# hanquansanren/DvD

Hardware: AMD Instinct MI355X
Metric: documents/sec (50-step DDIM, 288x288 grid) (higher is better)
Workload: dtype f16

## Files before the change

dvd_amd/csrc/tokens.hip:

```cpp
#include "common.h"
#include "mfma.h"

namespace dvd {

__device__ __forceinline__ float wave_sum(float v) {
#pragma unroll
  for (int o = 32; o > 0; o >>= 1) v += __shfl_xor(v, o);
  return v;
}

__global__ void __launch_bounds__(256) embed_obs_ln_kernel(const float* __restrict__ x, const float* __restrict__ w,
                                                           const float* __restrict__ bias,
                                                           const float* __restrict__ pos, float* __restrict__ tok32,
                                                           _Float16* __restrict__ ln16, int g, long rows) {
  const long row = (long)blockIdx.x * 4 + (threadIdx.x >> 6);
  if (row >= rows) return;
  const int lane = threadIdx.x & 63;
  const int side = g >> 1, T = side * side;
  const int n = (int)(row / T), t = (int)(row % T);
  const int ty = t / side, tx = t % side;
  float pv[8];
#pragma unroll
  for (int c = 0; c < 2; ++c)
#pragma unroll
    for (int p = 0; p < 2; ++p)
#pragma unroll
      for (int q = 0; q < 2; ++q)
        pv[c * 4 + p * 2 + q] = x[(((size_t)n * 2 + c) * g + (2 * ty + p)) * g + 2 * tx + q];
  float v[6];
  float s = 0.f;
#pragma unroll
  for (int j = 0; j < 6; ++j) {
    const int o = lane + 64 * j;
    float acc = bias[o];
#pragma unroll
    for (int k = 0; k < 8; ++k) acc += w[o * 8 + k] * pv[k];
    acc += pos[(size_t)t * 384 + o];
    v[j] = acc;
    s += acc;
  }
  const float mean = wave_sum(s) * (1.f / 384.f);
  float q2 = 0.f;
#pragma unroll
  for (int j = 0; j < 6; ++j) {
    const float d = v[j] - mean;
    q2 += d * d;
  }
  const float rstd = rsqrtf(wave_sum(q2) * (1.f / 384.f) + 1e-6f);
#pragma unroll
  for (int j = 0; j < 6; ++j) {
    const int o = lane + 64 * j;
    tok32[row * 384 + o] = v[j];
    ln16[row * 384 + o] = (_Float16)((v[j] - mean) * rstd);
  }
}

template <int C>
__global__ void __launch_bounds__(256) layernorm_rows_kernel(const float* __restrict__ in, int ldin, long sIn,
                                                             _Float16* __restrict__ out, int ldout, long sOut,
                                                             const float* __restrict__ gamma,
                                                             const float* __restrict__ beta,
                                                             const float* __restrict__ shift,
                                                             const float* __restrict__ scale, int ldmod,
                                                             int mod_rows, float eps, long rows) {
  constexpr int PER = C / 64;
  constexpr int V = (C == 384) ? 2 : 4;
  constexpr int NV = PER / V;
  const long row = (long)blockIdx.x * 4 + (threadIdx.x >> 6);
  if (row >= rows) return;
  const int lane = threadIdx.x & 63;
  const float* ip = in + blockIdx.y * sIn + row * ldin;
  float v[PER];
  float s = 0.f;
  typedef float fvec __attribute__((ext_vector_type(V)));
  typedef _Float16 hvec __attribute__((ext_vector_type(V)));
#pragma unroll
  for (int k = 0; k < NV; ++k) {
    const int c0 = (k * 64 + lane) * V;
    const fvec x = *(const fvec*)(ip + c0);
#pragma unroll
    for (int e = 0; e < V; ++e) {
      v[k * V + e] = x[e];
// ... 450 lines not shown
    }
  }
}

__global__ void __launch_bounds__(256) final_tokens_kernel(const float* __restrict__ z,
                                                           const float* __restrict__ gamma,
                                                           const float* __restrict__ beta,
                                                           const float* __restrict__ shift,
                                                           const float* __restrict__ scale, int ldmod,
                                                           int mod_rows, const float* __restrict__ w,
                                                           const float* __restrict__ b,
                                                           const float* __restrict__ init_flow,
                                                           float* __restrict__ x0, float* __restrict__ tok8, int g,
                                                           long rows) {
  constexpr int C = 1536, PER = 24;
  const long row = (long)blockIdx.x * 4 + (threadIdx.x >> 6);
  if (row >= rows) return;
  const int lane = threadIdx.x & 63;
  const float* ip = z + row * C;
  float v[PER];
  float s = 0.f;
#pragma unroll
  for (int k = 0; k < 6; ++k) {
    const floatx4 f = *(const floatx4*)(ip + (k * 64 + lane) * 4);
#pragma unroll
    for (int e = 0; e < 4; ++e) {
      v[k * 4 + e] = f[e];
      s += f[e];
    }
  }
  float mean = wave_sum(s) * (1.f / C);
  float q2 = 0.f;
#pragma unroll
  for (int k = 0; k < PER; ++k) {
    const float d = v[k] - mean;
    q2 += d * d;
  }
  float rstd = rsqrtf(wave_sum(q2) * (1.f / C) + 1e-5f);
  s = 0.f;
#pragma unroll
  for (int k = 0; k < 6; ++k)
#pragma unroll
    for (int e = 0; e < 4; ++e) {
      const int c = (k * 64 + lane) * 4 + e;
      v[k * 4 + e] = (v[k * 4 + e] - mean) * rstd * gamma[c] + beta[c];
      s += v[k * 4 + e];
    }
  mean = wave_sum(s) * (1.f / C);
  q2 = 0.f;
#pragma unroll
  for (int k = 0; k < PER; ++k) {
    const float d = v[k] - mean;
    q2 += d * d;
  }
  rstd = rsqrtf(wave_sum(q2) * (1.f / C) + 1e-6f);
  const float* sh = shift + (row / mod_rows) * ldmod;
  const float* sc = scale + (row / mod_rows) * ldmod;
  float dot[8];
#pragma unroll
  for (int j = 0; j < 8; ++j) dot[j] = 0.f;
#pragma unroll
  for (int k = 0; k < 6; ++k)
#pragma unroll
    for (int e = 0; e < 4; ++e) {
      const int c = (k * 64 + lane) * 4 + e;
      const float y = ((v[k * 4 + e] - mean) * rstd) * (1.f + sc[c]) + sh[c];
#pragma unroll
      for (int j = 0; j < 8; ++j) dot[j] += y * w[j * C + c];
    }
#pragma unroll
  for (int j = 0; j < 8; ++j) dot[j] = wave_sum(dot[j]);
  if (lane < 8) {
    float o = 0.f;
#pragma unroll
    for (int j = 0; j < 8; ++j)
      if (lane == j) o = dot[j];
    o += b[lane];
    if (tok8) tok8[row * 8 + lane] = o;
    const int side = g >> 1, T = side * side;
    const int n = (int)(row / T), t = (int)(row % T);
    const int p = lane >> 2, q = (lane >> 1) & 1, c = lane & 1;
    const size_t at = (((size_t)n * 2 + c) * g + 2 * (t / side) + p) * g + 2 * (t % side) + q;
    x0[at] = o + (init_flow ? init_flow[at] : 0.f);
  }
}

}

using namespace dvd;

#define LAUNCH_ROWS(rows) cdiv((rows), 4), 256, 0, (hipStream_t)stream

extern "C" int dvd_embed_obs_ln(const float* x, const float* w, const float* bias, const float* pos, float* tok32,
                                void* ln16, int n, int g, void* stream) {
  DVD_REQUIRE(x && w && bias && pos && tok32 && ln16, "embed_obs_ln: null pointer");
  DVD_REQUIRE(n > 0 && g >= 2 && g % 2 == 0, "embed_obs_ln: bad shape");
  const long rows = (long)n * (g / 2) * (g / 2);
  embed_obs_ln_kernel<<<LAUNCH_ROWS(rows)>>>(x, w, bias, pos, tok32, (_Float16*)ln16, g, rows);
  return check_launch("embed_obs_ln");
}

extern "C" int dvd_layernorm_rows(const float* in, int ldin, long stride_in, void* out16, int ldout, long stride_out,
                                  int batch, long rows, int c, const float* gamma, const float* beta,
                                  const float* shift, const float* scale, int ldmod, int mod_rows, float eps,
                                  void* stream) {
  DVD_REQUIRE(in && out16, "layernorm_rows: null pointer");
  DVD_REQUIRE(c == 384 || c == 1536, "layernorm_rows: C=%d not in {384,1536}", c);
  DVD_REQUIRE((gamma == nullptr) == (beta == nullptr) && (shift == nullptr) == (scale == nullptr),
              "layernorm_rows: affine / modulate pointers must come in pairs");
  DVD_REQUIRE(!shift || mod_rows > 0, "layernorm_rows: mod_rows");
  DVD_REQUIRE(rows > 0 && batch > 0 && batch < 65536, "layernorm_rows: bad rows/batch");
  DVD_REQUIRE(ldin % 4 == 0 && stride_in % 2 == 0 && ldout % 4 == 0 && stride_out % 2 == 0 && ldmod % 4 == 0 &&
                  ((uintptr_t)in % 16) == 0 && ((uintptr_t)out16 % 8) == 0 && ((uintptr_t)gamma % 16) == 0 &&
                  ((uintptr_t)beta % 16) == 0 && ((uintptr_t)shift % 16) == 0 && ((uintptr_t)scale % 16) == 0,
              "layernorm_rows: rows must be 16-byte aligned (vector loads)");
  dim3 grid(cdiv(rows, 4), batch);
  if (c == 384)
    layernorm_rows_kernel<384><<<grid, 256, 0, (hipStream_t)stream>>>(in, ldin, stride_in, (_Float16*)out16, ldout,
                                                                       stride_out, gamma, beta, shift, scale, ldmod,
                                                                       mod_rows > 0 ? mod_rows : 1, eps, rows);
  else
    layernorm_rows_kernel<1536><<<grid, 256, 0, (hipStream_t)stream>>>(in, ldin, stride_in, (_Float16*)out16, ldout,
                                                                        stride_out, gamma, beta, shift, scale, ldmod,
                                                                        mod_rows > 0 ? mod_rows : 1, eps, rows);
  return check_launch("layernorm_rows");
}

extern "C" int dvd_build_r_rows(const float* feat_nhwc, const float* init_feat_nchw, const float* flow, void* out16,
                                int ldo, int n, int g, int n_hyp, int mode, void* stream) {
  DVD_REQUIRE(feat_nhwc && flow && out16, "build_r_rows: null pointer");
  DVD_REQUIRE(ldo >= 1032 && n > 0 && g >= 2 && g % 2 == 0 && n_hyp > 0 && mode >= 0 && mode <= 3,
              "build_r_rows: bad arguments");
  DVD_REQUIRE(mode != 3 || init_feat_nchw, "build_r_rows: mode 3 needs init_feat");
  const long items = (long)n * (g / 2) * (g / 2) * 4;
  build_r_rows_kernel<<<LAUNCH_ROWS(items)>>>(feat_nhwc, init_feat_nchw, flow, (_Float16*)out16, ldo, g, n_hyp, mode,
                                              items);
  return check_launch("build_r_rows");
}

extern "C" int dvd_patch_rows(const float* in, long sn, long sc, long sy, long sx, float* out, int ldo, int n, int c,
                              int g, void* stream) {
  DVD_REQUIRE(in && out, "patch_rows: null pointer");
  DVD_REQUIRE(n > 0 && c > 0 && g >= 2 && g % 2 == 0 && ldo >= 4 * c, "patch_rows: bad shape");
  const long total = (long)n * (g / 2) * (g / 2) * 4 * c;
  patch_rows_kernel<<<cdiv(total, 256), 256, 0, (hipStream_t)stream>>>(in, sn, sc, sy, sx, out, ldo, c, g, total);
  return check_launch("patch_rows");
}

extern "C" int dvd_dwconv3x3(const void* in16, void* out16, const float* w9c, const float* b, int n, int side, int c,
                             void* stream) {
  DVD_REQUIRE(in16 && out16 && w9c && b, "dwconv3x3: null pointer");
  DVD_REQUIRE(n > 0 && side > 0 && c % 8 == 0, "dwconv3x3: bad shape");
#ifdef DVD_LAB
  if (getenv("DVD_DWCONV_V1")) {
    const long total1 = (long)n * side * side * (c / 8);
    dwconv3x3_kernel<<<cdiv(total1, 256), 256, 0, (hipStream_t)stream>>>((const _Float16*)in16, (_Float16*)out16, w9c, b,
                                                                         side, c, total1);
    return check_launch("dwconv3x3(lab v1)");
  }
#endif
  int stx = (c % 512 == 0 && (long)n * side * side >= 16384) ? 3 : 0, ssy = 24;
  bool snt = true;
  (void)snt;
#ifdef DVD_LAB
  if (getenv("DVD_DWCONV_TY") || getenv("DVD_DWCONV_TX")) stx = 0;
  if (const char* e = getenv("DVD_DWCONV_STRIP")) stx = (c % 512 == 0) ? atoi(e) : 0;
  if (const char* e = getenv("DVD_DWCONV_SY")) ssy = atoi(e);
  if (const char* e = getenv("DVD_DWCONV_NT")) snt = atoi(e) != 0;
#endif
  if (stx >= 2 && stx <= 4 && ssy >= 1) {
    const int xstrips = cdiv(side, stx), ybands = cdiv(side, ssy);
    const int nwaves = n * ybands * xstrips * (c / 512);
    const dim3 g(cdiv(nwaves, 4));
#define DW_STRIP(TX_, NT_) dwconv3x3_strip_kernel<TX_, NT_><<<g, 256, 0, (hipStream_t)stream>>>((const _Float16*)in16, (_Float16*)out16, w9c, b, side, c, ssy, xstrips, ybands, nwaves)
#ifdef DVD_LAB
    if (stx == 2) { if (snt) DW_STRIP(2, true); else DW_STRIP(2, false); }
    else if (stx == 4) { if (snt) DW_STRIP(4, true); else DW_STRIP(4, false); }
    else if (!snt) DW_STRIP(3, false);
    else
#endif
    DW_STRIP(3, true);
#undef DW_STRIP
    return check_launch("dwconv3x3(strip)");
  }
  int ty = DW_TY_P, tx = DW_TX_P;
#ifdef DVD_LAB
  if (const char* e = getenv("DVD_DWCONV_TY")) ty = atoi(e);
  if (const char* e = getenv("DVD_DWCONV_TX")) tx = atoi(e);
#endif
  const long total = (long)n * cdiv(side, ty) * cdiv(side, tx) * (c / 8);
  const dim3 grd(cdiv(total, 256));
#define DW_LAUNCH(TX_, TY_) dwconv3x3_tile_kernel<TX_, TY_><<<grd, 256, 0, (hipStream_t)stream>>>((const _Float16*)in16, (_Float16*)out16, w9c, b, side, c, total)
#ifdef DVD_LAB
  if (tx == 2 && ty == 2) DW_LAUNCH(2, 2);
  else if (tx == 2 && ty == 4) DW_LAUNCH(2, 4);
  else if (tx == 2 && ty == 8) DW_LAUNCH(2, 8);
  else if (tx == 1 && ty == 4) DW_LAUNCH(1, 4);
  else if (tx == 1 && ty == 8) DW_LAUNCH(1, 8);
  else if (tx == 2) DW_LAUNCH(2, 1);
  else if (ty == 1) DW_LAUNCH(4, 1);
  else if (ty == 4) DW_LAUNCH(4, 4);
  else
#endif
  DW_LAUNCH(DW_TX_P, DW_TY_P);
#undef DW_LAUNCH
  return check_launch("dwconv3x3");
}

extern "C" int dvd_colmean(const float* z, float* partial, float* pooled, int n, int t, int c, int chunks,
                           void* stream) {
  DVD_REQUIRE(z && partial && pooled, "colmean: null pointer");
  DVD_REQUIRE(n > 0 && n < 65536 && t > 0 && c > 0 && chunks > 0 && chunks < 65536, "colmean: bad shape");
  dim3 grid(cdiv(c, 256), chunks, n);
  colsum_partial_kernel<<<grid, 256, 0, (hipStream_t)stream>>>(z, partial, t, c, chunks);
  colmean_final_kernel<<<cdiv((long)n * c, 256), 256, 0, (hipStream_t)stream>>>(partial, pooled, t, c, chunks, n * c);
  return check_launch("colmean");
}

extern "C" int dvd_posenc_add(float* z, const float* hs, const float* ws, const float* htab, const float* wtab,
                              int n, int side, int c, void* stream) {
  DVD_REQUIRE(z && hs && ws && htab && wtab, "posenc_add: null pointer");
  DVD_REQUIRE(n > 0 && side > 0 && c % 4 == 0, "posenc_add: bad shape");
  const long total4 = (long)n * side * side * (c / 4);
  posenc_add_kernel<<<cdiv(total4, 256), 256, 0, (hipStream_t)stream>>>(z, hs, ws, htab, wtab, side, c, total4);
  return check_launch("posenc_add");
}

extern "C" int dvd_small_linear(const float* x, int ldx, const float* w, const float* b, float* y, int ldy, int m,
                                int k, int n, int kmod, int act_in, int act_out, void* stream) {
  DVD_REQUIRE(x && w && y, "small_linear: null pointer");
  DVD_REQUIRE(m > 0 && k > 0 && n > 0 && kmod > 0 && act_in >= 0 && act_in <= 2 && act_out >= 0 && act_out <= 3,
              "small_linear: bad arguments");
  small_linear_kernel<<<dim3(cdiv(n, 4), cdiv(m, 8)), 256, 0, (hipStream_t)stream>>>(x, ldx, w, b, y, ldy, m, k, n, kmod, act_in,
                                                                                       act_out);
  return check_launch("small_linear");
}

extern "C" int dvd_final_tokens(const float* z, const float* gamma, const float* beta, const float* shift,
                                const float* scale, int ldmod, int mod_rows, const float* w8, const float* b8,
                                const float* init_flow, float* x0, float* tok8, int n, int g, void* stream) {
  DVD_REQUIRE(z && gamma && beta && shift && scale && w8 && b8 && x0, "final_tokens: null pointer");
  DVD_REQUIRE(n > 0 && g >= 2 && g % 2 == 0 && mod_rows > 0, "final_tokens: bad shape");
  const long rows = (long)n * (g / 2) * (g / 2);
  final_tokens_kernel<<<LAUNCH_ROWS(rows)>>>(z, gamma, beta, shift, scale, ldmod, mod_rows, w8, b8, init_flow, x0,
                                             tok8, g, rows);
  return check_launch("final_tokens");
}
```

dvd_amd/lib.py:

```python
from __future__ import annotations

import ctypes as C
import os

import torch

_HERE = os.path.dirname(os.path.abspath(__file__))
LIB_PATH = os.path.join(_HERE, "libdvd_hip.so")


class DvdError(RuntimeError):
    pass


def _load():
    if not os.path.exists(LIB_PATH):
        raise DvdError(
            f"{LIB_PATH} is missing: build it with `python -c 'import __graft_entry__ as g; g.build()'` "
            "or `make -C dvd_amd/csrc`.  The DvD engine has no non-HIP fallback.")
    return C.CDLL(LIB_PATH)


_lib = _load()

# ... 30 lines not shown
                ("O", C.c_void_p), ("ldo", C.c_int), ("strideO", C.c_long),
                ("scale", C.c_float)]


class CnOp(C.Structure):
    _fields_ = [("op", C.c_int), ("a", C.c_int), ("b", C.c_int), ("dst", C.c_int), ("ks", C.c_int), ("dil", C.c_int),
                ("cout", C.c_int), ("act", C.c_int), ("w_off", C.c_long), ("h", C.c_int), ("w", C.c_int),
                ("flag", C.c_int)]


class RaggedImage(C.Structure):
    _fields_ = [("src", C.c_void_p), ("out", C.c_void_p), ("h", C.c_int), ("w", C.c_int)]


SSIM_REPLICATE, SSIM_VALID = 0, 1
MSSSIM_DOCUNET, MSSSIM_WANG = 0, 1

PNG_SEGMENT = 32768
PNG_HUFFMAN_FIXED, PNG_HUFFMAN_DYNAMIC = 0, 1

JPEG_420, JPEG_444 = 0, 1


class JpegDecInfo(C.Structure):
    _fields_ = [("h", C.c_int), ("w", C.c_int), ("out_h", C.c_int), ("out_w", C.c_int), ("components", C.c_int),
                ("hs", C.c_int), ("vs", C.c_int), ("orientation", C.c_int), ("restart_interval", C.c_int),
                ("scan_offset", C.c_long), ("scan_bytes", C.c_long), ("blocks", C.c_long), ("scratch_bytes", C.c_long)]


JPEG_DECODE_CODES = {-20: "HEADER", -21: "PROGRESSIVE", -22: "EXTENDED", -23: "LOSSLESS", -24: "ARITHMETIC", -25: "PRECISION",
                     -26: "COMPONENTS", -27: "ADOBE", -28: "SAMPLING", -29: "SCANS", -30: "QUANT16", -31: "TABLE", -32: "SIZE",
                     -33: "ORIENTATION", -34: "NOSYNC", -35: "DATA"}
JPEGDEC_SUBSEQ = 128

class SflowParams(C.Structure):
    _fields_ = [(name, C.c_int) for name in ("levels", "w_top", "w", "iters_top", "iters", "alpha", "d", "gamma", "T", "eps")]


SFLOW_DEFAULTS = dict(levels=4, w_top=10, w=2, iters_top=60, iters=30, alpha=510, d=10200, gamma=1, T=8160, eps=1 << 17)
SFLOW_MIN_TOP = 12

RAGGED_CAP = 64

NON_STATUS = {"dvd_last_error", "dvd_version", "dvd_engine_workspace_bytes", "dvd_engine_tensor_count",
              "dvd_flash_attn_kernel_name", "dvd_gemm_kernel_name", "dvd_convnet_workspace_bytes", "dvd_convnet_weight_floats",
              "dvd_ingest_scratch_bytes", "dvd_ingest_ragged_scratch_bytes", "dvd_resize_gray_scratch_bytes",
              "dvd_msssim_workspace_bytes", "dvd_png_bound", "dvd_png_scratch_bytes", "dvd_png_scratch_bytes_huff", "dvd_jpeg_bound",
              "dvd_jpeg_scratch_bytes", "dvd_sflow_level_workspace_bytes", "dvd_sflow_workspace_bytes",
              "dvd_adist_workspace_bytes"}

SIGNATURES = {
    "dvd_grid_sample_bilinear_zeros_ac": [c_void, c_void, c_void, C.c_int, C.c_int, C.c_int, C.c_int, C.c_int,
                                          C.c_int, C.c_int, c_void],
    "dvd_unwarp_f32": [c_void, C.c_int, c_void, c_void, C.c_int, C.c_int, C.c_float, c_void],
    "dvd_unwarp_u8": [c_void, C.c_int, c_void, c_void, C.c_int, C.c_int, C.c_float, c_void],
    "dvd_unwarp_f32_batch": [c_void, C.c_int, c_void, c_void, C.c_int, C.c_int, C.c_int, C.c_float, c_void],
    "dvd_unwarp_u8_batch": [c_void, C.c_int, c_void, c_void, C.c_int, C.c_int, C.c_int, C.c_float, c_void],
    "dvd_unwarp_grid": [c_void, C.c_int, c_void, C.c_int, C.c_int, C.c_float, c_void],
    "dvd_unwarp_u8_ragged": [c_void, C.c_int, C.POINTER(RaggedImage), C.c_int, C.c_float, c_void],
    "dvd_grid_sample_bicubic_zeros_ac": [c_void, c_void, c_void, C.c_int, C.c_int, C.c_int, C.c_int, C.c_int,
                                         C.c_int, C.c_int, c_void],
    "dvd_unwarp_u8_bicubic_batch": [c_void, C.c_int, c_void, c_void, C.c_int, C.c_int, C.c_int, C.c_float, c_void],
    "dvd_unwarp_u8_bicubic_ragged": [c_void, C.c_int, C.POINTER(RaggedImage), C.c_int, C.c_float, c_void],
    "dvd_sched_step": [C.POINTER(SchedCoef), c_void, c_void, c_void, c_void, c_void, C.c_int, C.c_int, c_void],
    "dvd_sched_step_clip": [C.POINTER(SchedCoef), c_void, c_void, c_void, c_void, c_void, C.c_int, C.c_int, c_void],
    "dvd_hyp_mean_clamp": [c_void, c_void, C.c_int, C.c_int, C.c_int, c_void],
    "dvd_selftest_mfma": [c_void, c_void, c_void, c_void, c_void],
    "dvd_gemm_nt": [C.POINTER(GemmDesc), c_void],
    "dvd_gemm_kernel_name": [C.POINTER(GemmDesc)],
    "dvd_flash_attn": [C.POINTER(AttnDesc), c_void],
    "dvd_embed_obs_ln": [c_void, c_void, c_void, c_void, c_void, c_void, C.c_int, C.c_int, c_void],
    "dvd_layernorm_rows": [c_void, C.c_int, C.c_long, c_void, C.c_int, C.c_long, C.c_int, C.c_long, C.c_int, c_void,
                           c_void, c_void, c_void, C.c_int, C.c_int, C.c_float, c_void],
    "dvd_build_r_rows": [c_void, c_void, c_void, c_void, C.c_int, C.c_int, C.c_int, C.c_int, C.c_int, c_void],
    "dvd_patch_rows": [c_void, C.c_long, C.c_long, C.c_long, C.c_long, c_void, C.c_int, C.c_int, C.c_int, C.c_int,
                       c_void],
    "dvd_dwconv3x3": [c_void, c_void, c_void, c_void, C.c_int, C.c_int, C.c_int, c_void],
    "dvd_colmean": [c_void, c_void, c_void, C.c_int, C.c_int, C.c_int, C.c_int, c_void],
    "dvd_posenc_add": [c_void, c_void, c_void, c_void, c_void, C.c_int, C.c_int, C.c_int, c_void],
    "dvd_small_linear": [c_void, C.c_int, c_void, c_void, c_void, C.c_int, C.c_int, C.c_int, C.c_int, C.c_int, C.c_int,
                         C.c_int, c_void],
    "dvd_final_tokens": [c_void, c_void, c_void, c_void, c_void, C.c_int, C.c_int, c_void, c_void, c_void, c_void,
                         c_void, C.c_int, C.c_int, c_void],
    "dvd_im2col3x3": [c_void, C.c_long, C.c_long, C.c_long, c_void, C.c_int, C.c_int, C.c_int, C.c_int, c_void],
    "dvd_conv3x3_nhwc": [c_void, C.c_int, c_void, C.c_int, c_void, c_void, C.c_int, C.c_int, C.c_int, C.c_int, c_void],
    "dvd_maxpool2_nhwc": [c_void, c_void, C.c_int, C.c_int, C.c_int, c_void],
    "dvd_resize_bilinear_nhwc": [c_void, c_void, C.c_int, C.c_int, C.c_int, C.c_int, C.c_int, c_void],
    "dvd_nhwc_to_nchw": [c_void, c_void, C.c_int, C.c_int, C.c_int, c_void],
    "dvd_convnet_create": [C.POINTER(CnOp), C.c_int, C.c_int, C.c_int, C.c_int, C.c_int, C.POINTER(c_void)],
    "dvd_convnet_create_batched": [C.POINTER(CnOp), C.c_int, C.c_int, C.c_int, C.c_int, C.c_int, C.c_int, C.POINTER(c_void)],
    "dvd_convnet_destroy": [c_void],
    "dvd_convnet_slot_shape": [c_void, C.c_int, C.POINTER(C.c_int), C.POINTER(C.c_int), C.POINTER(C.c_int)],
    "dvd_convnet_run": [c_void, c_void, c_void, c_void, C.c_long, C.c_int, C.POINTER(C.c_int), C.POINTER(c_void), c_void],
    "dvd_resize_bilinear_nchw": [c_void, c_void, C.c_long, C.c_int, C.c_int, C.c_int, C.c_int, C.c_int, c_void],
    "dvd_threshold_mask_mul": [c_void, c_void, c_void, c_void, C.c_int, C.c_long, C.c_float, c_void],
    "dvd_threshold_mask_mul_batch": [c_void, c_void, c_void, c_void, C.c_int, C.c_int, C.c_long, C.c_float, c_void],
    "dvd_flash_attn_f32": [C.POINTER(AttnDesc), c_void],
    "dvd_layernorm256_f32": [c_void, c_void, C.c_long, c_void, c_void, C.c_float, c_void],
    "dvd_add_rows_f32": [c_void, c_void, c_void, C.c_long, C.c_int, C.c_int, c_void],
    "dvd_transpose_f32": [c_void, c_void, C.c_int, C.c_int, C.c_int, c_void],
    "dvd_soft_mask_mul_batch": [c_void, c_void, c_void, C.c_int, C.c_int, C.c_long, c_void],
    "dvd_convex_upsample": [c_void, c_void, C.c_int, C.c_int, C.c_int, c_void, c_void, C.c_int, C.c_float, c_void],
    "dvd_ingest_u8": [c_void, C.c_int, C.c_int, C.c_int, c_void, C.c_int, c_void, c_void, c_void],
    "dvd_ingest_ragged_scratch_bytes": [C.c_int, C.c_int],
    "dvd_ingest_u8_ragged": [C.POINTER(RaggedImage), C.c_int, C.c_int, c_void, C.c_int, c_void, c_void],
    "dvd_resize_gray_scratch_bytes": [C.c_int, C.c_int, C.c_int, C.c_int],
    "dvd_resize_gray_u8": [c_void, C.c_int, C.c_int, C.c_int, c_void, C.c_int, C.c_int, c_void, c_void],
    "dvd_ssim_scale": [c_void, c_void, C.c_int, C.c_int, C.c_int, C.c_int, c_void, c_void],
    "dvd_ssim_finalize": [c_void, C.c_int, C.c_int, C.c_long, c_void, C.c_int, c_void],
    "dvd_reduce2_pair": [c_void, c_void, c_void, c_void, C.c_int, C.c_int, C.c_int, C.c_int, c_void],
    "dvd_msssim_workspace_bytes": [C.c_int, C.c_int, C.c_int],
    "dvd_msssim_scales": [c_void, c_void, C.c_int, C.c_int, C.c_int, C.c_int, c_void, c_void, c_void],
    "dvd_dsift_u8": [c_void, C.c_int, C.c_int, C.c_int, C.c_int, c_void, c_void],
    "dvd_sflow_cost": [c_void, c_void, c_void, C.c_int, C.c_int, C.c_int, C.POINTER(SflowParams), c_void, c_void],
    "dvd_sflow_level_workspace_bytes": [C.c_int, C.c_int, C.c_int],
    "dvd_sflow_level": [c_void, c_void, c_void, C.c_int, C.c_int, C.c_int, C.c_int, C.POINTER(SflowParams), c_void, c_void, c_void,
                        c_void],
    "dvd_sflow_workspace_bytes": [C.c_int, C.c_int, C.POINTER(SflowParams)],
    "dvd_sflow": [c_void, c_void, C.c_int, C.c_int, C.c_int, C.POINTER(SflowParams), c_void, c_void, c_void, c_void],
    "dvd_ad_fit": [c_void, C.c_int, C.c_int, C.c_int, c_void, c_void, c_void, c_void],
    "dvd_ad_align": [c_void, c_void, C.c_int, C.c_int, C.c_int, c_void, c_void],
    "dvd_ad_weighted": [c_void, c_void, C.c_int, C.c_int, C.c_int, c_void, c_void, c_void],
    "dvd_adist_workspace_bytes": [C.c_int, C.c_int, C.POINTER(SflowParams)],
    "dvd_adist": [c_void, c_void, C.c_int, C.c_int, C.c_int, C.POINTER(SflowParams), c_void, c_void, c_void, c_void, c_void, c_void,
                  c_void, c_void, c_void],
    "dvd_png_bound": [C.c_int, C.c_int],
    "dvd_png_scratch_bytes": [C.c_int, C.c_int],
    "dvd_png_encode_rgb8": [c_void, C.c_int, C.c_int, c_void, C.c_long, c_void, c_void, c_void],
    "dvd_png_scratch_bytes_huff": [C.c_int, C.c_int, C.c_int],
    "dvd_png_encode_rgb8_huff": [c_void, C.c_int, C.c_int, c_void, C.c_long, c_void, c_void, C.c_int, c_void],
    "dvd_jpeg_bound": [C.c_int, C.c_int, C.c_int],
    "dvd_jpeg_scratch_bytes": [C.c_int, C.c_int, C.c_int],
    "dvd_jpeg_encode_rgb8": [c_void, C.c_int, C.c_int, C.c_int, C.c_int, c_void, C.c_long, c_void, c_void, c_void],
    "dvd_jpegdec_probe": [c_void, C.c_long, C.POINTER(JpegDecInfo)],
    "dvd_jpeg_decode_rgb8": [c_void, c_void, C.c_long, c_void, C.c_long, C.c_int, C.POINTER(C.c_int), c_void, c_void],
    "dvd_dither_f16": [c_void, c_void, c_void, C.c_long, C.c_uint, C.c_uint, c_void],
    "dvd_engine_create": [C.c_int, C.c_int, C.c_int, C.POINTER(c_void)],
    "dvd_engine_destroy": [c_void],
    "dvd_engine_bind_workspace": [c_void, c_void, C.c_long],
    "dvd_engine_tensor_count": [c_void],
    "dvd_engine_tensor_info": [c_void, C.c_int, C.POINTER(C.c_char_p), C.POINTER(C.c_int), C.POINTER(C.c_long)],
    "dvd_engine_set_tensor": [c_void, C.c_char_p, c_void, C.c_long],
    "dvd_engine_prepare_docs": [c_void, c_void, c_void, c_void, c_void, c_void],
    "dvd_engine_feat_nchw": [c_void, c_void, c_void],
    "dvd_engine_denoise_step": [c_void, c_void, C.c_float, C.c_int, c_void, c_void, c_void, c_void],
    "dvd_engine_debug_buffer": [c_void, C.c_char_p, C.POINTER(c_void), C.POINTER(C.c_long)],
    "dvd_engine_debug_stop": [c_void, C.c_int],
    "dvd_engine_set_option": [c_void, C.c_char_p, C.c_int],
    "dvd_engine_profile": [c_void, C.c_int],
    "dvd_engine_profile_read": [c_void, C.POINTER(C.c_int), C.POINTER(C.c_double)],
}


RESTYPES = {"dvd_gemm_kernel_name": C.c_char_p, "dvd_ingest_ragged_scratch_bytes": C.c_long,
            "dvd_resize_gray_scratch_bytes": C.c_long, "dvd_msssim_workspace_bytes": C.c_long,
            "dvd_sflow_level_workspace_bytes": C.c_long, "dvd_sflow_workspace_bytes": C.c_long,
            "dvd_adist_workspace_bytes": C.c_long,
            "dvd_png_bound": C.c_long, "dvd_png_scratch_bytes": C.c_long, "dvd_png_scratch_bytes_huff": C.c_long,
            "dvd_jpeg_bound": C.c_long, "dvd_jpeg_scratch_bytes": C.c_long}

LAB_SIGNATURES = {"dvd_gemm_debug_stamps": [c_void], "dvd_attn_debug_stamps": [c_void]}


def bind(cdll):
    cdll.dvd_last_error.restype = C.c_char_p
    cdll.dvd_version.restype = C.c_int
# ... 56 lines not shown
```

dvd_amd/ops.py:

```python
from __future__ import annotations

import ctypes as C
import os

import numpy as np
import torch

from . import lib
from .lib import ptr, stream_ptr


def _chk(t: torch.Tensor, dtype, name):
    if not t.is_cuda:
        raise lib.DvdError(f"{name}: expected a device tensor (the DvD engine has no CPU path)")
    if t.dtype != dtype or not t.is_contiguous():
        raise lib.DvdError(f"{name}: expected contiguous {dtype}, got {t.dtype} contiguous={t.is_contiguous()}")


_WARP_MODES = ("bilinear", "bicubic")


def _warp_mode(mode, name):
    if mode not in _WARP_MODES:
        raise ValueError(f"{name}: mode must be 'bilinear' or 'bicubic', got {mode!r}")
# ... 177 lines not shown
    return None if t is None else t.data_ptr()


def gemm_nt(a, b, *, out32=None, out16=None, bias=None, bias_row=False, act=0, pos=None, gate=None,
            gate_rows=0, res=None, batch=1, strides=None, M=None, N=None, K=None, lda=None, ldb=None, b_lo=None,
            a_lo=None, lo_scale=2.0 ** -11, small_tiles=False):
    assert a.dtype == b.dtype and a.dtype in (torch.float16, torch.float32)
    d = lib.GemmDesc()
    d.dtype = 1 if a.dtype == torch.float32 else 0
    d.M = M if M is not None else a.shape[-2]
    d.N = N if N is not None else b.shape[-2]
    d.K = K if K is not None else a.shape[-1]
    d.batch = batch
    st = strides or {}
    d.A, d.lda, d.strideA = _addr(a), (lda if lda is not None else a.stride(-2)), st.get("A", 0)
    d.B, d.ldb, d.strideB = _addr(b), (ldb if ldb is not None else b.stride(-2)), st.get("B", 0)
    if b_lo is not None:
        d.B_lo, d.lo_scale = _addr(b_lo), lo_scale
    if a_lo is not None:
        d.A_lo, d.lo_scale = _addr(a_lo), lo_scale
    if out32 is not None:
        d.C32, d.ldc, d.strideC32 = _addr(out32), out32.stride(-2), st.get("C32", 0)
    if out16 is not None:
        d.C16, d.ldc16, d.strideC16 = _addr(out16), out16.stride(-2), st.get("C16", 0)
    if bias is not None:
        d.bias, d.bias_row, d.strideBias = _addr(bias), int(bias_row), st.get("bias", 0)
    d.act = act
    if pos is not None:
        d.pos, d.ldpos, d.pos_rows = _addr(pos), pos.stride(-2), pos.shape[-2]
    if gate is not None:
        d.gate, d.ldgate, d.gate_rows, d.strideGate = _addr(gate), gate.stride(-2), gate_rows, st.get("gate", 0)
    if res is not None:
        d.res, d.ldres, d.strideRes = _addr(res), res.stride(-2), st.get("res", 0)
    d.small_tiles = int(small_tiles)
    lib.call("dvd_gemm_nt", C.byref(d), stream_ptr())


def flash_attn(q, k, vt, out, heads, head_dim, scale, kv_batch_div=1):
    d = lib.AttnDesc()
    d.head_dim, d.heads, d.batch, d.tq, d.tk = head_dim, heads, q.shape[0], q.shape[1], k.shape[1]
    d.kv_batch_div = kv_batch_div
    d.Q, d.ldq, d.strideQ = q.data_ptr(), q.stride(1), q.stride(0)
    d.K, d.ldk, d.strideK = k.data_ptr(), k.stride(1), k.stride(0)
    d.Vt, d.ldvt, d.strideVt = vt.data_ptr(), vt.stride(1), vt.stride(0)
    d.O, d.ldo, d.strideO = out.data_ptr(), out.stride(1), out.stride(0)
    d.scale = scale
    lib.call("dvd_flash_attn", C.byref(d), stream_ptr())
    return out


def layernorm_rows(x, c, gamma=None, beta=None, shift=None, scale=None, mod_rows=1, eps=1e-6):
    rows = x.shape[0]
    out = torch.empty(rows, c, dtype=torch.float16, device=x.device)
    lib.call("dvd_layernorm_rows", ptr(x), x.stride(0), 0, ptr(out), c, 0, 1, rows, c, ptr(gamma), ptr(beta), ptr(shift),
             ptr(scale), (shift.stride(0) if shift is not None and shift.dim() > 1 else 0), mod_rows, C.c_float(eps),
             stream_ptr())
    return out


def dwconv3x3(x16, w9c, b, n, side):
    out = torch.empty_like(x16)
    lib.call("dvd_dwconv3x3", ptr(x16), ptr(out), ptr(w9c), ptr(b), n, side, x16.shape[-1], stream_ptr())
    return out


def embed_obs_ln(x, w, b, pos):
    n, _, g, _ = x.shape
    T = (g // 2) ** 2
    tok = torch.empty(n * T, 384, dtype=torch.float32, device=x.device)
    ln = torch.empty(n * T, 384, dtype=torch.float16, device=x.device)
    lib.call("dvd_embed_obs_ln", ptr(x), ptr(w), ptr(b), ptr(pos), ptr(tok), ptr(ln), n, g, stream_ptr())
    return tok, ln


def small_linear(x, w, b, act_in=0, act_out=0, kmod=None):
    m = x.shape[0]
    n, k = w.shape
    y = torch.empty(m, n, dtype=torch.float32, device=x.device)
    lib.call("dvd_small_linear", ptr(x), x.stride(0), ptr(w), ptr(b), ptr(y), n, m, k, n, kmod or k, act_in, act_out,
             stream_ptr())
    return y


def final_tokens(z, gamma, beta, shift, scale, w8, b8, init_flow, n, g):
    x0 = torch.empty(n, 2, g, g, dtype=torch.float32, device=z.device)
    tok8 = torch.empty(z.shape[0], 8, dtype=torch.float32, device=z.device)
    lib.call("dvd_final_tokens", ptr(z), ptr(gamma), ptr(beta), ptr(shift), ptr(scale), 0, z.shape[0], ptr(w8), ptr(b8),
             ptr(init_flow), ptr(x0), ptr(tok8), n, g, stream_ptr())
    return x0, tok8


def posenc(z, hs, ws, htab, wtab, n, side):
    c = z.shape[-1]
    chunks = 8
    part = torch.empty(n * chunks * c, dtype=torch.float32, device=z.device)
    pooled = torch.empty(n, c, dtype=torch.float32, device=z.device)
    lib.call("dvd_colmean", ptr(z), ptr(part), ptr(pooled), n, side * side, c, chunks, stream_ptr())
    lib.call("dvd_posenc_add", ptr(z), ptr(hs), ptr(ws), ptr(htab), ptr(wtab), n, side, c, stream_ptr())
    return pooled


def build_r_rows(feat_nhwc, flow, n_hyp, mode, init_feat=None):
    n, _, g, _ = flow.shape
    T = (g // 2) ** 2
    out = torch.empty(n * T, 1088, dtype=torch.float16, device=flow.device)
    lib.call("dvd_build_r_rows", ptr(feat_nhwc), ptr(init_feat), ptr(flow), ptr(out), 1088, n, g, n_hyp, mode, stream_ptr())
    return out


def conv3x3_relu_nhwc(x_nhwc, w_packed, bias, cin, cout, h, w):
    kp = w_packed.shape[1]
    col = torch.empty(h * w, kp, dtype=torch.float32, device=x_nhwc.device)
    lib.call("dvd_im2col3x3", ptr(x_nhwc), 1, w * cin, cin, ptr(col), kp, cin, h, w, stream_ptr())
    out = torch.empty(h * w, cout, dtype=torch.float32, device=x_nhwc.device)
    gemm_nt(col, w_packed, out32=out, bias=bias, act=2)
    return out


def conv3x3_relu_nhwc_implicit(x_nhwc, w_packed, bias, cin, cout, h, w):
    out = torch.empty(h * w, cout, dtype=torch.float32, device=x_nhwc.device)
    lib.call("dvd_conv3x3_nhwc", ptr(x_nhwc), cin, ptr(w_packed), w_packed.shape[1], ptr(bias), ptr(out), cout, h, w, 1,
             stream_ptr())
    return out


def maxpool2_nhwc(x, c, h, w):
    out = torch.empty((h // 2) * (w // 2), c, dtype=torch.float32, device=x.device)
    lib.call("dvd_maxpool2_nhwc", ptr(x), ptr(out), c, h, w, stream_ptr())
    return out


def resize_bilinear_nhwc(x, c, hin, win, hout, wout):
    out = torch.empty(hout * wout, c, dtype=torch.float32, device=x.device)
    lib.call("dvd_resize_bilinear_nhwc", ptr(x), ptr(out), c, hin, win, hout, wout, stream_ptr())
    return out


MSSSIM_WEIGHTS = (0.0448, 0.2856, 0.3001, 0.2363, 0.1333)
MSSSIM_MIN_SIDE = 176
MSSSIM_AREA = 598400
_SSIM_PRESETS = {"docunet": lib.MSSSIM_DOCUNET, "wang": lib.MSSSIM_WANG}


def _ssim_preset(preset, name):
    if preset not in _SSIM_PRESETS:
        raise ValueError(f"{name}: preset must be 'docunet' or 'wang', got {preset!r}")
    return _SSIM_PRESETS[preset]


def _size_query(name, *args):
    nbytes = getattr(lib.raw(), name)(*args)
    if nbytes < 0:
        raise lib.DvdError(f"{name} failed ({nbytes}): {lib.raw().dvd_last_error().decode()}")
    return nbytes


def resize_gray_u8(img_nhwc_u8: torch.Tensor, out_h: int, out_w: int) -> torch.Tensor:
    if img_nhwc_u8.dim() != 4 or img_nhwc_u8.shape[0] < 1 or img_nhwc_u8.shape[3] != 3:
        raise ValueError(f"resize_gray_u8: expected [N,H,W,3] with N >= 1, got {tuple(img_nhwc_u8.shape)}")
    n, h, w, _ = img_nhwc_u8.shape
    if min(h, w, out_h, out_w) < 1:
        raise ValueError(f"resize_gray_u8: bad shape {h}x{w} -> {out_h}x{out_w}")
    _chk(img_nhwc_u8, torch.uint8, "img")
    out = torch.empty((n, out_h, out_w), dtype=torch.float32, device=img_nhwc_u8.device)
    scratch = torch.empty(_size_query("dvd_resize_gray_scratch_bytes", h, w, out_h, out_w), dtype=torch.uint8,
                          device=img_nhwc_u8.device)
    lib.call("dvd_resize_gray_u8", ptr(img_nhwc_u8), n, h, w, ptr(out), out_h, out_w, ptr(scratch), stream_ptr())
    return out


def ssim_scales(x: torch.Tensor, y: torch.Tensor, preset: str = "docunet") -> torch.Tensor:
# ... 485 lines not shown
```

include/dvd_hip.h:

```cpp
#ifndef DVD_HIP_H
#define DVD_HIP_H

#include <stddef.h>
#include <stdint.h>

#ifdef __cplusplus
extern "C" {
#endif

#define DVD_OK 0
#define DVD_E_ARG (-1)
#define DVD_E_LAUNCH (-2)
#define DVD_E_STATE (-3)

const char* dvd_last_error(void);
int dvd_version(void);


int dvd_grid_sample_bilinear_zeros_ac(const float* src, const float* grid, float* out,
                                      int n, int c, int hin, int win, int h, int w,
                                      int src_batch_div, void* stream);

int dvd_unwarp_f32(const float* flow, int g, const float* src_chw, float* out_hwc,
                   int h, int w, float scale, void* stream);
// ... 16 lines not shown
                                     int n, int c, int hin, int win, int h, int w,
                                     int src_batch_div, void* stream);
int dvd_unwarp_u8_bicubic_batch(const float* flow, int g, const uint8_t* src_hwc, uint8_t* out_hwc,
                                int n, int h, int w, float scale, void* stream);
int dvd_unwarp_u8_bicubic_ragged(const float* flow, int g, const dvd_ragged_image* docs, int n, float scale, void* stream);

typedef struct {
  int kind;
  float c_recip;
  float c_recipm1;
  float sqrt_abar_prev;
  float dir_coef;
  float coef1;
  float coef2;
  float sigma;
} dvd_sched_coef;

int dvd_sched_step(const dvd_sched_coef* coef, const float* x_t, const float* x0, const float* noise,
                   float* x_prev, float* next_grid, int n, int g, void* stream);

int dvd_sched_step_clip(const dvd_sched_coef* coef, const float* x_t, float* x0, const float* noise,
                        float* x_prev, float* next_grid, int n, int g, void* stream);

int dvd_hyp_mean_clamp(const float* x0, float* out, int docs, int n_hyp, int g, void* stream);

typedef struct {
  int dtype;
  int M, N, K, batch;
  const void* A; int lda; long strideA;
  const void* B; int ldb; long strideB;
  const void* B_lo; const void* A_lo; float lo_scale;
  float* C32; int ldc; long strideC32;
  void* C16; int ldc16; long strideC16;
  const float* bias; int bias_row; long strideBias;
  int act;
  const float* pos; int ldpos; int pos_rows;
  const float* gate; int ldgate; int gate_rows; long strideGate;
  const float* res; int ldres; long strideRes;
  int small_tiles;
} dvd_gemm_desc;

int dvd_gemm_nt(const dvd_gemm_desc* desc, void* stream);
const char* dvd_gemm_kernel_name(const dvd_gemm_desc* desc);

typedef struct {
  int head_dim, heads, batch, tq, tk, kv_batch_div;
  const void* Q; int ldq; long strideQ;
  const void* K; int ldk; long strideK;
  const void* Vt; int ldvt; long strideVt;
  void* O; int ldo; long strideO;
  float scale;
} dvd_attn_desc;

int dvd_flash_attn(const dvd_attn_desc* desc, void* stream);
const char* dvd_flash_attn_kernel_name(int head_dim, int tq, int tk);


int dvd_embed_obs_ln(const float* x, const float* w, const float* bias, const float* pos, float* tok32,
                     void* ln16, int n, int g, void* stream);

int dvd_layernorm_rows(const float* in, int ldin, long stride_in, void* out16, int ldout, long stride_out,
                       int batch, long rows, int c, const float* gamma, const float* beta, const float* shift,
                       const float* scale, int ldmod, int mod_rows, float eps, void* stream);

int dvd_build_r_rows(const float* feat_nhwc, const float* init_feat_nchw, const float* flow, void* out16, int ldo,
                     int n, int g, int n_hyp, int mode, void* stream);

int dvd_patch_rows(const float* in, long sn, long sc, long sy, long sx, float* out, int ldo, int n, int c, int g,
                   void* stream);

int dvd_dwconv3x3(const void* in16, void* out16, const float* w9c, const float* b, int n, int side, int c,
                  void* stream);

int dvd_colmean(const float* z, float* partial, float* pooled, int n, int t, int c, int chunks, void* stream);
int dvd_posenc_add(float* z, const float* hs, const float* ws, const float* htab, const float* wtab, int n, int side,
                   int c, void* stream);

int dvd_small_linear(const float* x, int ldx, const float* w, const float* b, float* y, int ldy, int m, int k, int n,
                     int kmod, int act_in, int act_out, void* stream);

int dvd_final_tokens(const float* z, const float* gamma, const float* beta, const float* shift, const float* scale,
                     int ldmod, int mod_rows, const float* w8, const float* b8, const float* init_flow, float* x0,
                     float* tok8, int n, int g, void* stream);

int dvd_im2col3x3(const float* in, long sc, long sy, long sx, float* out, int ldo, int c, int h, int w, void* stream);
int dvd_conv3x3_nhwc(const float* in, int c, const float* wgt, int kp, const float* bias, float* out, int cout, int h, int w,
                     int relu, void* stream);
int dvd_maxpool2_nhwc(const float* in, float* out, int c, int h, int w, void* stream);
int dvd_resize_bilinear_nhwc(const float* in, float* out, int c, int hin, int win, int hout, int wout, void* stream);
int dvd_nhwc_to_nchw(const float* in, float* out, int c, int h, int w, void* stream);

enum { DVD_CN_CONV = 0, DVD_CN_POOL = 1, DVD_CN_RESIZE = 2, DVD_CN_ADD = 3, DVD_CN_SIGMOID = 4, DVD_CN_INSTNORM = 5 };
typedef struct {
  int op;
  int a, b;
  int dst;
  int ks, dil;
  int cout, act;
  long w_off;
  int h, w;
  int flag;
} dvd_cn_op;

int dvd_convnet_create(const dvd_cn_op* ops, int n_ops, int n_slots, int in_c, int in_h, int in_w, void** handle);
int dvd_convnet_create_batched(const dvd_cn_op* ops, int n_ops, int n_slots, int in_c, int in_h, int in_w, int batch,
                               void** handle);
int dvd_convnet_destroy(void* handle);
long dvd_convnet_workspace_bytes(void* handle);
long dvd_convnet_weight_floats(void* handle);
int dvd_convnet_slot_shape(void* handle, int slot, int* h, int* w, int* c);
int dvd_convnet_run(void* handle, const float* in_nchw, const float* weights, void* workspace, long workspace_bytes,
                    int n_out, const int* out_slots, float* const* out_nchw, void* stream);
int dvd_resize_bilinear_nchw(const float* in, float* out, long planes, int hin, int win, int hout, int wout,
                             int align_corners, void* stream);
int dvd_threshold_mask_mul(const float* d0, const float* x_nchw, float* out_nchw, float* mask_out, int c, long hw,
                           float thr, void* stream);
int dvd_threshold_mask_mul_batch(const float* d0, const float* x_nchw, float* out_nchw, float* mask_out, int n, int c,
                                 long hw, float thr, void* stream);

int dvd_flash_attn_f32(const dvd_attn_desc* desc, void* stream);
int dvd_layernorm256_f32(const float* in, float* out, long rows, const float* gamma, const float* beta, float eps,
                         void* stream);
int dvd_add_rows_f32(const float* a, const float* pos, float* out, long rows, int pos_rows, int c, void* stream);
int dvd_transpose_f32(const float* in, float* out, int n, int rows, int cols, void* stream);
int dvd_soft_mask_mul_batch(const float* msk, const float* x_nchw, float* out_nchw, int n, int c, long hw, void* stream);
int dvd_convex_upsample(const float* mask, const float* dflow, int n, int h, int w, float* bm, float* init_flow, int g,
                        float norm, void* stream);

long dvd_ingest_scratch_bytes(int out_size);
int dvd_ingest_u8(const uint8_t* src_hwc, int h, int w, int swap_rb, float* y_chw, int out_size,
                  uint8_t* rgb_hwc_out, void* scratch, void* stream);

long dvd_ingest_ragged_scratch_bytes(int out_size, int n);
int dvd_ingest_u8_ragged(const dvd_ragged_image* docs, int n, int swap_rb, float* y_nchw, int out_size, void* scratch,
                         void* stream);

int dvd_dither_f16(const void* hi, const void* lo, void* out, long nelem, unsigned elem0, unsigned step, void* stream);

int dvd_engine_create(int grid, int docs, int n_hyp, void** handle);
int dvd_engine_destroy(void* handle);
long dvd_engine_workspace_bytes(void* handle);
int dvd_engine_bind_workspace(void* handle, void* workspace, long bytes);
int dvd_engine_tensor_count(void* handle);
int dvd_engine_tensor_info(void* handle, int index, const char** name, int* dtype , long* nelem);
int dvd_engine_set_tensor(void* handle, const char* name, const void* dev_ptr, long nelem);
int dvd_engine_set_option(void* handle, const char* name, int value);
int dvd_engine_prepare_docs(void* handle, const float* y512, const float* mask_cat, const float* mask_y512,
                            const float* line_msk, void* stream);
int dvd_engine_feat_nchw(void* handle, float* out, void* stream);
int dvd_engine_denoise_step(void* handle, const float* x_t, float t_embed, int feat_mode, const float* init_flow,
                            const float* init_feat_nchw , float* x0_out, void* stream);
int dvd_engine_profile(void* handle, int enable);
int dvd_engine_profile_read(void* handle, int* launches, double* total_ms);
int dvd_engine_debug_buffer(void* handle, const char* name, void** ptr, long* bytes);
int dvd_engine_debug_stop(void* handle, int stage);

int dvd_selftest_mfma(const void* a16, const void* b16, const void* vt16, float* out3072, void* stream);

#define DVD_SSIM_REPLICATE 0
#define DVD_SSIM_VALID 1
#define DVD_MSSSIM_DOCUNET 0
#define DVD_MSSSIM_WANG 1
long dvd_resize_gray_scratch_bytes(int h, int w, int out_h, int out_w);
int dvd_resize_gray_u8(const uint8_t* src_nhwc, int n, int h, int w, float* out, int out_h, int out_w,
                       void* scratch, void* stream);
int dvd_ssim_scale(const float* x, const float* y, int n, int h, int w, int border, double* partials, void* stream);
// ... 93 lines not shown
```

Before: 0.4894.

## Add persistent two-rows-per-wave final_tokens kernel with LDS-staged projection weights

Adds a persistent grid-stride kernel for the final double-LayerNorm plus 8-way projection. Each wave handles two rows packed into float2 vectors, and the 8x1536 weight matrix is staged once per block in shared memory instead of being re-read from global memory for every row. It is selected by default when pointers are 16-byte aligned, with the old kernel kept as a fallback. The Python wrapper now also passes the real shift stride instead of 0. The cost is higher register pressure and a hardcoded C=1536, and the kernel is a small slice of a 50-step diffusion pipeline.

```diff
diff --git a/dvd_amd/csrc/tokens.hip b/dvd_amd/csrc/tokens.hip
--- a/dvd_amd/csrc/tokens.hip
+++ b/dvd_amd/csrc/tokens.hip
@@ -1,3 +1,5 @@
+#include <algorithm>
+
 #include "common.h"
 #include "mfma.h"
 
@@ -614,6 +616,116 @@
     const int p = lane >> 2, q = (lane >> 1) & 1, c = lane & 1;
     const size_t at = (((size_t)n * 2 + c) * g + 2 * (t / side) + p) * g + 2 * (t % side) + q;
     x0[at] = o + (init_flow ? init_flow[at] : 0.f);
+  }
+}
+
+typedef float floatx2 __attribute__((ext_vector_type(2)));
+__global__ void __launch_bounds__(256, 3) final_tokens_stream_kernel(const float* __restrict__ z,
+                                                                  const float* __restrict__ gamma,
+                                                                  const float* __restrict__ beta,
+                                                                  const float* __restrict__ shift,
+                                                                  const float* __restrict__ scale, int ldmod,
+                                                                  int mod_rows, const float* __restrict__ w,
+                                                                  const float* __restrict__ b,
+                                                                  const float* __restrict__ init_flow,
+                                                                  float* __restrict__ x0, float* __restrict__ tok8,
+                                                                  int g, int rows) {
+  constexpr int C = 1536, PER = 24, R = 2;
+  __shared__ __attribute__((aligned(16))) float wl[8 * C];
+  for (int i = threadIdx.x; i < 8 * C / 4; i += 256) ((floatx4*)wl)[i] = ((const floatx4*)w)[i];
+  __syncthreads();
+  const int lane = threadIdx.x & 63, wave = threadIdx.x >> 6;
+  const int ngroups = (rows + 4 * R - 1) / (4 * R);
+  for (int grp = blockIdx.x; grp < ngroups; grp += gridDim.x) {
+    const int row0 = (grp * 4 + wave) * R;
+    if (row0 >= rows) continue;
+    floatx2 v[PER];
+    const float *sc[R], *sh[R];
+    {
+      floatx4 f[R][6];
+#pragma unroll
+      for (int i = 0; i < R; ++i) {
+        const int row = min(row0 + i, rows - 1);
+        const unsigned mod = (unsigned)row / (unsigned)mod_rows;
+        sc[i] = scale + (size_t)mod * ldmod;
+        sh[i] = shift + (size_t)mod * ldmod;
+#pragma unroll
+        for (int k = 0; k < 6; ++k) f[i][k] = *(const floatx4*)(z + (size_t)row * C + (k * 64 + lane) * 4);
+      }
+#pragma unroll
+      for (int k = 0; k < 6; ++k)
+#pragma unroll
+        for (int e = 0; e < 4; ++e) v[k * 4 + e] = floatx2{f[0][k][e], f[1][k][e]};
+    }
+    floatx2 s = {0.f, 0.f};
+#pragma unroll
+    for (int k = 0; k < PER; ++k) s += v[k];
+    floatx2 mean = floatx2{wave_sum(s[0]), wave_sum(s[1])} * (1.f / C);
+    floatx2 q2 = {0.f, 0.f};
+#pragma unroll
+    for (int k = 0; k < PER; ++k) {
+      const floatx2 d = v[k] - mean;
+      q2 += d * d;
+    }
+    floatx2 rstd = {rsqrtf(wave_sum(q2[0]) * (1.f / C) + 1e-5f), rsqrtf(wave_sum(q2[1]) * (1.f / C) + 1e-5f)};
+    s = floatx2{0.f, 0.f};
+#pragma unroll
+    for (int k = 0; k < 6; ++k) {
+      const floatx4 g4 = *(const floatx4*)(gamma + (k * 64 + lane) * 4), b4 = *(const floatx4*)(beta + (k * 64 + lane) * 4);
+#pragma unroll
+      for (int e = 0; e < 4; ++e) {
+        v[k * 4 + e] = (v[k * 4 + e] - mean) * rstd * g4[e] + b4[e];
+        s += v[k * 4 + e];
+      }
+    }
+    mean = floatx2{wave_sum(s[0]), wave_sum(s[1])} * (1.f / C);
+    q2 = floatx2{0.f, 0.f};
+#pragma unroll
+    for (int k = 0; k < PER; ++k) {
+      const floatx2 d = v[k] - mean;
+      q2 += d * d;
+    }
+    rstd = floatx2{rsqrtf(wave_sum(q2[0]) * (1.f / C) + 1e-6f), rsqrtf(wave_sum(q2[1]) * (1.f / C) + 1e-6f)};
+    floatx2 dot[8];
+#pragma unroll
+    for (int j = 0; j < 8; ++j) dot[j] = floatx2{0.f, 0.f};
+#pragma unroll
+    for (int k = 0; k < 6; ++k) {
+      floatx4 w4[8];
+#pragma unroll
+      for (int j = 0; j < 8; ++j) w4[j] = *(const floatx4*)(wl + j * C + (k * 64 + lane) * 4);
+      const floatx4 sc0 = *(const floatx4*)(sc[0] + (k * 64 + lane) * 4), sh0 = *(const floatx4*)(sh[0] + (k * 64 + lane) * 4);
+      const floatx4 sc1 = *(const floatx4*)(sc[1] + (k * 64 + lane) * 4), sh1 = *(const floatx4*)(sh[1] + (k * 64 + lane) * 4);
+#pragma unroll
+      for (int e = 0; e < 4; ++e) {
+        const floatx2 y = ((v[k * 4 + e] - mean) * rstd) * (1.f + floatx2{sc0[e], sc1[e]}) + floatx2{sh0[e], sh1[e]};
+#pragma unroll
+        for (int j = 0; j < 8; ++j) dot[j] += y * w4[j][e];
+      }
+      __builtin_amdgcn_sched_barrier(0);
+    }
+    float red[R][8];
+#pragma unroll
+    for (int i = 0; i < R; ++i)
+#pragma unroll
+      for (int j = 0; j < 8; ++j) red[i][j] = wave_sum(dot[j][i]);
+#pragma unroll
+    for (int i = 0; i < R; ++i) {
+      const int row = row0 + i;
+      if (lane < 8 && row < rows) {
+        float o = 0.f;
+#pragma unroll
+        for (int j = 0; j < 8; ++j)
+          if (lane == j) o = red[i][j];
+        o += b[lane];
+        if (tok8) tok8[(size_t)row * 8 + lane] = o;
+        const int side = g >> 1, T = side * side;
+        const int n = (int)((unsigned)row / (unsigned)T), t = (int)((unsigned)row % (unsigned)T);
+        const int p = lane >> 2, q = (lane >> 1) & 1, c = lane & 1;
+        const size_t at = (((size_t)n * 2 + c) * g + 2 * (t / side) + p) * g + 2 * (t % side) + q;
+        x0[at] = o + (init_flow ? init_flow[at] : 0.f);
+      }
+    }
   }
 }
 
@@ -768,13 +880,32 @@
   return check_launch("small_linear");
 }
 
+extern "C" int dvd_final_tokens_form(const float* z, const float* gamma, const float* beta, const float* shift,
+                                     const float* scale, int ldmod, int mod_rows, const float* w8, const float* b8,
+                                     const float* init_flow, float* x0, float* tok8, int n, int g, int form,
+                                     void* stream) {
+  DVD_REQUIRE(z && gamma && beta && shift && scale && w8 && b8 && x0, "final_tokens: null pointer");
+  DVD_REQUIRE(n > 0 && g >= 2 && g % 2 == 0 && mod_rows > 0, "final_tokens: bad shape");
+  DVD_REQUIRE(form >= 0 && form <= 2, "final_tokens: form %d not in {0,1,2}", form);
+  const long rows = (long)n * (g / 2) * (g / 2);
+  auto a16 = [](const void* q) { return ((uintptr_t)q % 16) == 0; };
+  const bool aligned = a16(z) && a16(gamma) && a16(beta) && a16(shift) && a16(scale) && a16(w8) && ldmod % 4 == 0;
+  DVD_REQUIRE(form != 2 || aligned, "final_tokens: the streaming kernel needs 16-byte aligned z / gamma / beta / shift / scale / w8");
+  const bool fits = rows < (1L << 31) - 8 && (g / 2) * (g / 2) > 0;
+  DVD_REQUIRE(form != 2 || fits, "final_tokens: the streaming kernel takes fewer than 2^31 - 8 rows");
+  if (form == 1 || (form == 0 && !(aligned && fits))) {
+    final_tokens_kernel<<<LAUNCH_ROWS(rows)>>>(z, gamma, beta, shift, scale, ldmod, mod_rows, w8, b8, init_flow, x0,
+                                               tok8, g, rows);
+    return check_launch("final_tokens");
+  }
+  const long groups = cdiv(rows, 8);
+  final_tokens_stream_kernel<<<(unsigned)std::min<long>(groups, 768), 256, 0, (hipStream_t)stream>>>(
+      z, gamma, beta, shift, scale, ldmod, mod_rows, w8, b8, init_flow, x0, tok8, g, (int)rows);
+  return check_launch("final_tokens(stream)");
+}
+
 extern "C" int dvd_final_tokens(const float* z, const float* gamma, const float* beta, const float* shift,
                                 const float* scale, int ldmod, int mod_rows, const float* w8, const float* b8,
                                 const float* init_flow, float* x0, float* tok8, int n, int g, void* stream) {
-  DVD_REQUIRE(z && gamma && beta && shift && scale && w8 && b8 && x0, "final_tokens: null pointer");
-  DVD_REQUIRE(n > 0 && g >= 2 && g % 2 == 0 && mod_rows > 0, "final_tokens: bad shape");
-  const long rows = (long)n * (g / 2) * (g / 2);
-  final_tokens_kernel<<<LAUNCH_ROWS(rows)>>>(z, gamma, beta, shift, scale, ldmod, mod_rows, w8, b8, init_flow, x0,
-                                             tok8, g, rows);
-  return check_launch("final_tokens");
-}
+  return dvd_final_tokens_form(z, gamma, beta, shift, scale, ldmod, mod_rows, w8, b8, init_flow, x0, tok8, n, g, 0, stream);
+}
diff --git a/dvd_amd/lib.py b/dvd_amd/lib.py
--- a/dvd_amd/lib.py
+++ b/dvd_amd/lib.py
@@ -136,6 +136,8 @@
                          C.c_int, c_void],
     "dvd_final_tokens": [c_void, c_void, c_void, c_void, c_void, C.c_int, C.c_int, c_void, c_void, c_void, c_void,
                          c_void, C.c_int, C.c_int, c_void],
+    "dvd_final_tokens_form": [c_void, c_void, c_void, c_void, c_void, C.c_int, C.c_int, c_void, c_void, c_void, c_void,
+                              c_void, C.c_int, C.c_int, C.c_int, c_void],
     "dvd_im2col3x3": [c_void, C.c_long, C.c_long, C.c_long, c_void, C.c_int, C.c_int, C.c_int, C.c_int, c_void],
     "dvd_conv3x3_nhwc": [c_void, C.c_int, c_void, C.c_int, c_void, c_void, C.c_int, C.c_int, C.c_int, C.c_int, c_void],
     "dvd_maxpool2_nhwc": [c_void, c_void, C.c_int, C.c_int, C.c_int, c_void],
diff --git a/dvd_amd/ops.py b/dvd_amd/ops.py
--- a/dvd_amd/ops.py
+++ b/dvd_amd/ops.py
@@ -283,11 +283,16 @@
     return y
 
 
-def final_tokens(z, gamma, beta, shift, scale, w8, b8, init_flow, n, g):
+def final_tokens(z, gamma, beta, shift, scale, w8, b8, init_flow, n, g, form=None, mod_rows=None):
     x0 = torch.empty(n, 2, g, g, dtype=torch.float32, device=z.device)
     tok8 = torch.empty(z.shape[0], 8, dtype=torch.float32, device=z.device)
-    lib.call("dvd_final_tokens", ptr(z), ptr(gamma), ptr(beta), ptr(shift), ptr(scale), 0, z.shape[0], ptr(w8), ptr(b8),
-             ptr(init_flow), ptr(x0), ptr(tok8), n, g, stream_ptr())
+    ldmod = shift.stride(0) if shift.dim() > 1 else 0
+    args = (ptr(z), ptr(gamma), ptr(beta), ptr(shift), ptr(scale), ldmod, mod_rows or z.shape[0], ptr(w8), ptr(b8),
+            ptr(init_flow), ptr(x0), ptr(tok8), n, g)
+    if form is None:
+        lib.call("dvd_final_tokens", *args, stream_ptr())
+    else:
+        lib.call("dvd_final_tokens_form", *args, form, stream_ptr())
     return x0, tok8
 
 
diff --git a/include/dvd_hip.h b/include/dvd_hip.h
--- a/include/dvd_hip.h
+++ b/include/dvd_hip.h
@@ -122,6 +122,9 @@
 int dvd_final_tokens(const float* z, const float* gamma, const float* beta, const float* shift, const float* scale,
                      int ldmod, int mod_rows, const float* w8, const float* b8, const float* init_flow, float* x0,
                      float* tok8, int n, int g, void* stream);
+int dvd_final_tokens_form(const float* z, const float* gamma, const float* beta, const float* shift, const float* scale,
+                          int ldmod, int mod_rows, const float* w8, const float* b8, const float* init_flow, float* x0,
+                          float* tok8, int n, int g, int form, void* stream);
 
 int dvd_im2col3x3(const float* in, long sc, long sy, long sx, float* out, int ldo, int c, int h, int w, void* stream);
 int dvd_conv3x3_nhwc(const float* in, int c, const float* wgt, int kp, const float* bias, float* out, int cout, int h, int w,
```

Result: no change. 0.4899 (median of 6 runs) (+0.1%).
